# robert80203/HuPR-A-Benchmark-for-Human-Pose-Estimation-Using-Millimeter-Wave-Radar

Hardware: AMD Instinct MI355X
Metric: radar frames/sec (FFT->heatmap fwd+bwd) (higher is better)
Workload: dtype bf16

## Files before the change

### hupr-a-benchmark-for-human-pose-estimation-using-millimeter-wave-radar_amd/csrc/conv_halo256m_bf16.hip

```cpp
#include "conv_halo.h"

namespace hupr {

typedef float f32x4c __attribute__((ext_vector_type(4)));

template <int TD, int TH, int TW, int KD, int NCOT = 0, int NWN = 2, int KC = 64, bool TP = false>
__global__ __launch_bounds__(512) void hupr_k_conv_halo256m_bf16(HaloArgs p) {
    constexpr int LDK = KC, BN = 32 * NWN, TS = KC == 64 ? 3 : 9, C8 = KC / 8, L2C8 = KC == 64 ? 3 : 2;
    static_assert(KC == 64 || (KC == 32 && KD == 3 && NWN == 2 && NCOT == 0), "32-channel rows: 3 x 3 x 3 taps, 64 output channels per tile");
    static_assert(!TP || (TD == 2 && KD == 3 && NWN == 2 && KC == 64), "two-plane form: the 2 x 8 x 16 tile at D == 2 (launcher: nd == 1)");
    constexpr int NIMG = TP ? 2 * TS : TS;
    constexpr int HD = TP ? TD : TD + KD - 1, HH = TH + 2, HW = TW + 2;
    static_assert(TD * TH * TW == 64 * (8 / NWN) && TH % 8 == 0 && TW % 8 == 0 && (KD == 1 || KD == 3) && (NWN == 2 || NCOT == 0),
                  "256 (512) voxels per tile, 8 x 8 per wave");
    constexpr int NVOX = HD * HH * HW;
    constexpr int T = 9 * KD, NSTAGE = TP ? 6 : (KC == 64 ? 3 * KD : KD), NTAP = KC == 64 ? 6 : 9;
    constexpr bool FULLD = NWN == 1;
    constexpr int NVOXL = FULLD ? TD * HH * HW : NVOX, VOX0 = FULLD ? HH * HW : 0;
    constexpr int NH = (NVOXL * C8 + 511) / 512;
    constexpr int Y0 = NH < NTAP - 1 ? NH : NTAP - 1, Y1 = NH - (NTAP - 1) < 0 ? 0 : (NH - (NTAP - 1) > NTAP ? NTAP : NH - (NTAP - 1)),
                  Y2 = NH - (2 * NTAP - 1) < 0 ? 0 : (NH - (2 * NTAP - 1) > NTAP ? NTAP : NH - (2 * NTAP - 1));
    static_assert(NH <= NTAP * NSTAGE - 1 && NH <= 3 * NTAP - 1, "halo items must all be issued in front of the item's last barrier (and within three stages)");
    __shared__ __attribute__((aligned(16))) __bf16 Hs[(KC == 32 ? 2 : 1) * NVOX * LDK];
    __shared__ __attribute__((aligned(16))) __bf16 Bs[2][NIMG][BN * LDK];
    constexpr bool STATS = NCOT > 0 && KD == 3;
    constexpr bool SINGLE = STATS && TD == 2;
    f32x4c ssum[STATS ? NCOT : 1][2], ssq[STATS ? NCOT : 1][2];
    if constexpr (!SINGLE) {
#pragma unroll
        for (int ct = 0; ct < (STATS ? NCOT : 1); ++ct)
#pragma unroll
            for (int cg = 0; cg < 2; ++cg) { ssum[ct][cg] = (f32x4c){0.f, 0.f, 0.f, 0.f}; ssq[ct][cg] = (f32x4c){0.f, 0.f, 0.f, 0.f}; }
    }

    const int tid = threadIdx.x, lane = tid & 63, wave = tid >> 6;
    if (wave >= 4) __builtin_amdgcn_s_setprio(1);
    const int wm = NWN == 2 ? wave >> 1 : wave, wn = NWN == 2 ? wave & 1 : 0;
    constexpr int NBX = TW / 8, NBY = TH / 8;
    const int xw0 = 8 * (wm % NBX), yw0 = 8 * ((wm / NBX) % NBY), dzw = wm / (NBX * NBY);
    const int idx = lane & 15, kq = lane >> 4, yy = idx >> 3, wx = idx & 7;
    const int n_tiles = p.Bn * p.nd * p.nh * p.nw * p.n_co_tiles;

    const int wrow_ = NWN == 2 ? 8 * wave + (lane >> 3) : ((8 * wave + (lane >> 3)) & 31);
    const int wsrc_lane = (wrow_ * T * p.Ci + (((lane & 7) ^ (wrow_ >> 1)) & 7) * 8) * 2 +
                          (NWN == 2 ? 0 : (wave >> 2) * (3 * p.Ci * 2));
    constexpr int NDMA = NWN == 2 ? NIMG : 2, DMA_TAPS = NWN == 2 ? 1 : 2;
    const int wrow32_ = 16 * (wave & 3) + (lane >> 2);
    const int wsrc32_lane = (wrow32_ * T * p.Ci + (((lane & 3) ^ (((wrow32_ >> 3) & 1) << 1)) & 3) * 8) * 2;
    const u32x4 wrs = {(unsigned)(unsigned long)p.wp, (unsigned)((unsigned long)p.wp >> 32) & 0xffffu,
                       (unsigned)((long)p.Co * T * p.Ci * 2), 0x00020000u};
    const unsigned bs_lds = (unsigned)(unsigned long)(__attribute__((address_space(3))) void*)&Bs[0][0][0];
    const unsigned wdst_wave = __builtin_amdgcn_readfirstlane(bs_lds + wave * 1024);
#define HUPR_W_DMA(COT_, CH_, S_, PAR_)                                                                             \
    if constexpr (KC == 32) {                                                                                       \
        _Pragma("unroll") for (int j = 0; j < 5; ++j) {                                                             \
            if (j < 4 || wave < 4) {                                                                                \
                const int t9_ = 2 * j + (wave >> 2);                                  \
                const int wb32_ = (((COT_) * BN * T + (S_) * 9 + (t9_ % 3) * 3 + t9_ / 3) * p.Ci + (CH_) * KC) * 2 + wsrc32_lane; \
                unsigned keep_;                                                                                     \
                asm volatile("s_mov_b32 %0, m0\n\ts_mov_b32 m0, %1\n\ts_nop 0\n\tbuffer_load_dwordx4 %2, %3, 0 offen lds\n\t" \
                             "s_mov_b32 m0, %0"                                                                     \
                             : "=&s"(keep_)                                                                         \
                             : "s"(wdst_wave + (PAR_) * TS * (BN * LDK * 2) + j * 8192), "v"(wb32_), "s"(wrs)       \
                             : "memory");                                                                           \
            }                                                                                                       \
        }                                                                                                           \
    } else {                                                                                                        \
        const int wbase_ = (((COT_) * BN * T + ((S_) / 3) * 9 + ((S_) % 3)) * p.Ci + (CH_) * KC) * 2 + wsrc_lane;   \
        _Pragma("unroll") for (int j = 0; j < NDMA; ++j) {                                                          \
            if (NWN == 2 || j == 0 || wave < 4) {                                                                   \
                 \
                               \
                const int tap_ = (j < 3 ? 9 : 0) + 3 * (j % 3);                                                     \
                unsigned keep_;                                                                                     \
                asm volatile("s_mov_b32 %0, m0\n\ts_mov_b32 m0, %1\n\ts_nop 0\n\tbuffer_load_dwordx4 %2, %3, 0 offen lds\n\t" \
                             "s_mov_b32 m0, %0"                                                                     \
                             : "=&s"(keep_)                                                                         \
                             : "s"(NWN == 2 ? wdst_wave + ((PAR_) * NIMG + j) * (BN * LDK * 2)                      \
                                            : wdst_wave + (PAR_) * TS * (BN * LDK * 2) + j * 8192),                 \
                               "v"(TP ? wbase_ + tap_ * (p.Ci * 2)                                                  \
                                      : (NWN == 2 ? wbase_ + j * (3 * p.Ci * 2) : wbase_ + j * DMA_TAPS * (3 * p.Ci * 2))), "s"(wrs) \
                             : "memory");                                                                           \
            }                                                                                                       \
        }                                                                                                           \
    }

    u32x4 vb[NH];
    const __amdgpu_buffer_rsrc_t xrs = __builtin_amdgcn_make_buffer_rsrc(
        const_cast<void*>(p.x), 0, (int)((long)p.Bn * p.D * p.H * p.W * p.in_ld * 2), 0x00020000);
#define HUPR_HALO_ISSUE_ITEM(u, COND_, B_, D0_, H0_, W0_, C0_)                                                     \
    {                                                                                                               \
        const int it = tid + (u) * 512;                                                                             \
        const int vox = it >> L2C8, c8 = it & (C8 - 1);                                                             \
        const int hx = vox % HW;                                                                                    \
        const int t_ = vox / HW;                                                                                    \
        const int hy = t_ % HH, hz = t_ / HH;                                                                       \
        const int d = (D0_) + hz - (FULLD || TP ? 0 : KD / 2), h = (H0_) + hy - 1, w = (W0_) + hx - 1;                    \
        const bool ok = (COND_) && it < NVOXL * C8 && (unsigned)d < (unsigned)p.D && (unsigned)h < (unsigned)p.H && \
                        (unsigned)w < (unsigned)p.W;                                                                \
        const int off = (((((B_) * p.D + d) * p.H + h) * p.W + w) * p.in_ld + (C0_) + c8 * 8) * 2;                  \
        const auto ld_ = __builtin_amdgcn_raw_buffer_load_b128(xrs, ok ? off : 0x7ffffff0, 0, 0);                  \
        vb[u] = (u32x4){ld_[0], ld_[1], ld_[2], ld_[3]};                                                            \
    }
#define HUPR_HALO_COMMIT()                                                                                          \
    _Pragma("unroll") for (int u = 0; u < NH; ++u) {                                                                \
        const int it = tid + u * 512;                                                                               \
        if (it < NVOXL * C8) {                                                                                      \
            const int vox = it >> L2C8, c8 = it & (C8 - 1);                                                         \
            const int hx = vox % HW;                                                                                \
            const int key_ = KC == 64 ? (((hx >> 1) & 3) << 1) : ((((vox / HW) % HH) & 1) << 1);                    \
            *reinterpret_cast<u32x4*>(&Hs[(vox + VOX0) * LDK + ((c8 ^ key_) << 3)]) = vb[u];                        \
        }                                                                                                           \
    }

    struct Pos { int cot, twi, thi, tdi, b, ch; };
    const int n_chunks = p.Ci / KC;
    const int per_wg = (n_tiles + gridDim.x - 1) / gridDim.x;
    const int wg_rank = (int)((blockIdx.x & 7) * (gridDim.x >> 3) + (blockIdx.x >> 3));
    const int t_begin = wg_rank * per_wg, t_end = min(n_tiles, t_begin + per_wg);
    if (STATS && p.stats) {
        if (t_begin >= t_end) {
            for (int c = tid; c < 2 * p.Co; c += 512) p.stats[(long)blockIdx.x * 2 * p.Co + c] = 0.0;
        }
    }
    if (t_begin >= t_end) return;
    Pos cur;
    {
        cur.cot = t_begin % p.n_co_tiles;
        int st = t_begin / p.n_co_tiles;
        cur.twi = st % p.nw; st /= p.nw;
        cur.thi = st % p.nh; st /= p.nh;
        cur.tdi = st % p.nd;
        cur.b = st / p.nd;
        cur.ch = 0;
    }
    const int n_items = (t_end - t_begin) * n_chunks;
    const int cot0 = cur.cot;

    int woff[2][2];
#pragma unroll
    for (int cg = 0; cg < 2; ++cg)
#pragma unroll
        for (int kk = 0; kk < 2; ++kk) {
            const int n = 32 * wn + 16 * cg + idx;
            woff[cg][kk] = KC == 64 ? n * LDK + (((4 * kk + kq) ^ ((n >> 1) & 7)) << 3) : n * LDK + ((kq ^ (((n >> 3) & 1) << 1)) << 3);
            if constexpr (TP) woff[cg][kk] += dzw * (TS * BN * LDK);
        }
    const int xlane = (((TP ? 0 : dzw) * HH + yw0 + yy) * HW + xw0 + wx) * LDK;
#define HUPR_HALO_COMMIT1(u, HW_)                                                                                   \
    {                                                                                                               \
        const int it = tid + (u) * 512;                                                                             \
        if (it < NVOXL * C8) {                                                                                      \
            const int vox = it >> L2C8, c8 = it & (C8 - 1);                                                         \
            const int key_ = (((vox / HW) % HH) & 1) << 1;                                                          \
            *reinterpret_cast<u32x4*>(&Hs[(HW_) + (vox + VOX0) * LDK + ((c8 ^ key_) << 3)]) = vb[u];                \
        }                                                                                                           \
    }
#define HUPR_XF(ST_, RHO_, KK_)                                                                                     \
    (KC == 64 ? *reinterpret_cast<const bf16x8*>(&Hs[xlane + ((((ST_) / 3) * HH + (RHO_)) * HW + ((ST_) % 3)) * LDK + \
                    (((4 * (KK_) + kq) ^ ((((xw0 + wx + ((ST_) % 3)) >> 1) & 3) << 1)) << 3)])                      \
              : *reinterpret_cast<const bf16x8*>(&Hs[hrd + xlane + (((ST_) * HH + (RHO_)) * HW + (KK_)) * LDK +     \
                    ((kq ^ (((yy + (RHO_)) & 1) << 1)) << 3)]))
#define HUPR_WF(BUF_, KY_, CG_, KK_)                                                                                \
    (TP ? *reinterpret_cast<const bf16x8*>(&Bs[0][0][0] + ((BUF_) * NIMG + (KY_)) * (BN * LDK) + woff[CG_][KK_])    \
     : KC == 64 ? *reinterpret_cast<const bf16x8*>(&Bs[BUF_][KY_][woff[CG_][KK_]])                                  \
              : *reinterpret_cast<const bf16x8*>(&Bs[BUF_][3 * (KK_) + (KY_)][woff[CG_][0]]))

    f32x4c c[4][2];
    unsigned accP[4][2][2];
    __bf16* pP = nullptr;
    bool pend = false;
    constexpr bool RESPF = !STATS && TD != 2 && NWN == 2;
    const bool res_pf = RESPF && p.res != nullptr && (p.res_ld & 3) == 0 && !p.no_res_prefetch;
    constexpr bool BIASPF = KC == 32;
    const bool defer = (!p.bias || BIASPF) && (!p.res || res_pf) && (p.Co & 7) == 0 && (p.out_ld & 7) == 0;
    float biasv[BIASPF ? 2 : 1][4];
    bf16x4 resv[4][2];
    constexpr int NB = KC == 64 ? 2 : 3;
    bf16x8 xq[NB][4], x8, wq[NB][2];
#define HUPR_LOAD_TAP(ST_, TAU_, BUF_, WX_)                                                                         \
    {                                                                                                               \
        constexpr int kk_ = (TAU_) / 3, ky_ = (TAU_) % 3;                                                           \
        if ((WX_) & 1) {                                                                                            \
            wq[(TAU_) % NB][0] = HUPR_WF(BUF_, ky_, 0, kk_);                                                        \
            wq[(TAU_) % NB][1] = HUPR_WF(BUF_, ky_, 1, kk_);                                                        \
        }                                                                                                           \
        if ((WX_) & 2) {                                                                                            \
            if (ky_ == 0) { _Pragma("unroll") for (int vg = 0; vg < 4; ++vg) xq[kk_ % NB][vg] = HUPR_XF(ST_, 2 * vg, kk_); } \
            else if (ky_ == 1) { _Pragma("unroll") for (int vg = 0; vg < 4; ++vg) xq[(kk_ + 1) % NB][vg] = HUPR_XF(ST_, 2 * vg + 1, kk_); } \
            else { x8 = HUPR_XF(ST_, 8, kk_); }                                                                     \
        }                                                                                                           \
    }
#define HUPR_VMCNT_LGKM0(N_) __builtin_amdgcn_s_waitcnt(0x0070 | ((N_) & 15) | (((N_) >> 4) << 14))

    if constexpr (FULLD) {
        for (int i = tid; i < 2 * HH * HW * C8; i += 512) {
            const int pl = i / (HH * HW * C8), r = i - pl * (HH * HW * C8);
            *reinterpret_cast<u32x4*>(&Hs[pl * (HD - 1) * HH * HW * LDK + r * 8]) = (u32x4){0u, 0u, 0u, 0u};
        }
    }
    HUPR_W_DMA(cur.cot, cur.ch, 0, 0)
    HUPR_W_DMA(cur.cot, cur.ch, 1, 1)
#pragma unroll
    for (int u = 0; u < NH; ++u) HUPR_HALO_ISSUE_ITEM(u, true, cur.b, cur.tdi * TD, cur.thi * TH, cur.twi * TW, cur.ch * KC)
    [[maybe_unused]] int hrd = 0;
    if constexpr (KC == 32) {
#pragma unroll
        for (int u = 0; u < NH; ++u) HUPR_HALO_COMMIT1(u, 0)
    } else {
        HUPR_HALO_COMMIT()
    }
    __builtin_amdgcn_s_waitcnt(0x0F70);
    __syncthreads();
    HUPR_LOAD_TAP(0, 0, 0, 3)

    int g = 0;
    for (int q = 0; q < n_items; ++q) {
        const int b = cur.b, d0 = cur.tdi * TD, h0 = cur.thi * TH, w0 = cur.twi * TW, n0 = cur.cot * BN;
        const bool first_chunk = cur.ch == 0, last_chunk = cur.ch == n_chunks - 1;
        Pos nxt = cur;
        if (++nxt.ch == n_chunks) {
            nxt.ch = 0;
            if (++nxt.cot == p.n_co_tiles) {
                nxt.cot = 0;
                if (++nxt.twi == p.nw) {
                    nxt.twi = 0;
                    if (++nxt.thi == p.nh) {
                        nxt.thi = 0;
                        if (++nxt.tdi == p.nd) { nxt.tdi = 0; ++nxt.b; }
                    }
                }
            }
        }
        const bool has_next = q + 1 < n_items;
        if constexpr (KC == 32) hrd = (q & 1) * (NVOX * LDK);
        [[maybe_unused]] const int hwr = NVOX * LDK - hrd;
        if (first_chunk) {
#pragma unroll
            for (int vg = 0; vg < 4; ++vg)
#pragma unroll
                for (int cg = 0; cg < 2; ++cg) c[vg][cg] = (f32x4c){0.f, 0.f, 0.f, 0.f};
            if constexpr (BIASPF) {
                if (p.bias && defer) {
#pragma unroll
                    for (int cg = 0; cg < 2; ++cg)
#pragma unroll
                        for (int r = 0; r < 4; ++r) biasv[cg][r] = p.bias[n0 + 32 * wn + 16 * cg + 4 * kq + r];
                }
            }
        }
#pragma unroll
        for (int st_ = 0; st_ < NSTAGE; ++st_) {
            const int par = TP ? (st_ & 1) : ((g + st_) & 1);
#pragma unroll
            for (int tau = 0; tau < NTAP; ++tau) {
                const int kk = tau / 3, ky = tau % 3;
                if (tau == NTAP - 1) {
                    if (st_ == 0) { if (pend) { HUPR_VMCNT_LGKM0(Y0 + 4); } else { HUPR_VMCNT_LGKM0(Y0); } }
                    else if (st_ == 1) { HUPR_VMCNT_LGKM0(Y1); }
                    else if (st_ == 2) { HUPR_VMCNT_LGKM0(Y2); }
                    else { HUPR_VMCNT_LGKM0(0); }
                    __syncthreads();
                    if (st_ + 2 < NSTAGE) { HUPR_W_DMA(cur.cot, cur.ch, st_ + 2, par) }
                    else if (has_next) { HUPR_W_DMA(nxt.cot, nxt.ch, st_ + 2 - NSTAGE, par) }
                    if (KC == 64 && st_ == NSTAGE - 1 && has_next) { HUPR_HALO_COMMIT() }
                }
                if (tau == 0) { HUPR_LOAD_TAP(st_, 1, par, 3) }
                else if (tau == 1) { HUPR_LOAD_TAP(st_, 2, par, 3) }
                else if (tau == 2) { HUPR_LOAD_TAP(st_, 3, par, 3) }
                else if (tau == 3) { HUPR_LOAD_TAP(st_, 4, par, 3) }
                else if (tau == 4) { HUPR_LOAD_TAP(st_, 5, par, 3) }
                else if (NTAP == 9 && tau == 5) { if constexpr (NTAP == 9) { HUPR_LOAD_TAP(st_, 6, par, 3) } }
                else if (NTAP == 9 && tau == 6) { if constexpr (NTAP == 9) { HUPR_LOAD_TAP(st_, 7, par, 3) } }
                else if (NTAP == 9 && tau == 7) { if constexpr (NTAP == 9) { HUPR_LOAD_TAP(st_, 8, par, 3) } }
                else if (st_ + 1 < NSTAGE) { HUPR_LOAD_TAP((st_ + 1) % NSTAGE, 0, par ^ 1, 3) }
                else if (has_next) {
                    if constexpr (KC == 32) { const int hrd = hwr; HUPR_LOAD_TAP(0, 0, par ^ 1, 3) }
                    else { HUPR_LOAD_TAP(0, 0, par ^ 1, 1) }
                }
#pragma unroll
                for (int vg = 0; vg < 4; ++vg) {
                    const bf16x8 xf = ky == 0 ? xq[kk % NB][vg] : (ky == 1 ? xq[(kk + 1) % NB][vg] : (vg < 3 ? xq[kk % NB][vg + 1] : x8));
                    c[vg][0] = __builtin_amdgcn_mfma_f32_16x16x32_bf16(wq[tau % NB][0], xf, c[vg][0], 0, 0, 0);
                    c[vg][1] = __builtin_amdgcn_mfma_f32_16x16x32_bf16(wq[tau % NB][1], xf, c[vg][1], 0, 0, 0);
                }
                if (st_ == 0 && pend && tau < 4) {
                    const auto r0 = __builtin_amdgcn_permlane16_swap(accP[tau][0][0], accP[tau][1][0], false, false);
                    const auto r1 = __builtin_amdgcn_permlane16_swap(accP[tau][0][1], accP[tau][1][1], false, false);
                    *reinterpret_cast<u32x4*>(pP + (long)(2 * tau * p.W) * p.out_ld) = (u32x4){r0[0], r1[0], r0[1], r1[1]};
                }
                if (RESPF && st_ == NSTAGE - 1 && tau == 0) {
                    if (res_pf && last_chunk && defer) {
                        const long mr = (((long)b * p.D + d0 + dzw) * p.H + h0 + yw0 + yy) * p.W + w0 + xw0 + wx;
                        const int chr = n0 + 32 * wn + 4 * kq;
#pragma unroll
                        for (int vg = 0; vg < 4; ++vg)
#pragma unroll
                            for (int cg = 0; cg < 2; ++cg)
                                resv[vg][cg] = *reinterpret_cast<const bf16x4*>(static_cast<const __bf16*>(p.res) + (mr + 2 * vg * p.W) * p.res_ld +
                                                                                chr + 16 * cg);
                    }
                }
                if constexpr (KC == 32) {
                    if (st_ == NSTAGE - 1 && tau < NH && has_next) { HUPR_HALO_COMMIT1(tau, hwr) }
                }
                if (NTAP * st_ + tau < NH) {
                    HUPR_HALO_ISSUE_ITEM(NTAP * st_ + tau, has_next, nxt.b, nxt.tdi * TD, nxt.thi * TH, nxt.twi * TW, nxt.ch * KC)
                }
                __builtin_amdgcn_sched_group_barrier(0x100, 1, 0);
                __builtin_amdgcn_sched_group_barrier(0x008, 2, 0);
                __builtin_amdgcn_sched_group_barrier(0x100, 1, 0);
                __builtin_amdgcn_sched_group_barrier(0x008, 2, 0);
#pragma unroll
                for (int i_ = 0; i_ < 4; ++i_) {
                    __builtin_amdgcn_sched_group_barrier(0x100, 1, 0);
                    __builtin_amdgcn_sched_group_barrier(0x008, 1, 0);
                }
                __builtin_amdgcn_sched_barrier(0);
            }
            if (st_ == 0) pend = false;
        }
        g += NSTAGE;
        if (last_chunk) {
            const long m0 = (((long)b * p.D + d0 + dzw) * p.H + h0 + yw0 + yy) * p.W + w0 + xw0 + wx;
            const int ch0 = n0 + 32 * wn + 4 * kq;
            typedef __bf16 bf16x2 __attribute__((ext_vector_type(2)));
            if (defer && has_next) {
                if constexpr (BIASPF) {
                    if (p.bias) {
#pragma unroll
                        for (int vg = 0; vg < 4; ++vg)
#pragma unroll
                            for (int cg = 0; cg < 2; ++cg)
#pragma unroll
                                for (int r = 0; r < 4; ++r) c[vg][cg][r] += biasv[cg][r];
                    }
                }
                if (RESPF && res_pf) {
#pragma unroll
                    for (int vg = 0; vg < 4; ++vg)
#pragma unroll
                        for (int cg = 0; cg < 2; ++cg)
#pragma unroll
                            for (int r = 0; r < 4; ++r) c[vg][cg][r] += (float)resv[vg][cg][r];
                }
#pragma unroll
                for (int vg = 0; vg < 4; ++vg)
#pragma unroll
                    for (int cg = 0; cg < 2; ++cg) {
                        const bf16x2 lo = {(__bf16)c[vg][cg][0], (__bf16)c[vg][cg][1]}, hi = {(__bf16)c[vg][cg][2], (__bf16)c[vg][cg][3]};
                        accP[vg][cg][0] = __builtin_bit_cast(unsigned, lo);
                        accP[vg][cg][1] = __builtin_bit_cast(unsigned, hi);
                    }
                pP = static_cast<__bf16*>(p.y) + m0 * p.out_ld + n0 + 32 * wn + ((kq & 1) ? 16 + 4 * (kq - 1) : 4 * kq);
                pend = true;
            } else {
#pragma unroll
                for (int vg = 0; vg < 4; ++vg)
#pragma unroll
                    for (int cg = 0; cg < 2; ++cg) {
                        const long m = m0 + 2 * vg * p.W;
                        const int ch = ch0 + 16 * cg;
                        if (ch < p.Co) {
                            f32x4n v = {c[vg][cg][0], c[vg][cg][1], c[vg][cg][2], c[vg][cg][3]};
                            if (p.bias) v += (f32x4n){p.bias[ch], p.bias[ch + 1], p.bias[ch + 2], p.bias[ch + 3]};
                            if (p.res) {
                                const bf16x4 rv = *reinterpret_cast<const bf16x4*>(static_cast<const __bf16*>(p.res) + m * p.res_ld + ch);
                                v += (f32x4n){(float)rv[0], (float)rv[1], (float)rv[2], (float)rv[3]};
                            }
                            const bf16x4 o = {(__bf16)v[0], (__bf16)v[1], (__bf16)v[2], (__bf16)v[3]};
                            *reinterpret_cast<bf16x4*>(static_cast<__bf16*>(p.y) + m * p.out_ld + ch) = o;
                        }
                    }
            }
            if (STATS && p.stats) {
                int li = cur.cot - cot0;
                li += li < 0 ? p.n_co_tiles : 0;
                if constexpr (SINGLE) {
#pragma unroll
                    for (int cg = 0; cg < 2; ++cg) {
                        f32x4c sv = {0.f, 0.f, 0.f, 0.f}, qv = sv;
#pragma unroll
                        for (int vg = 0; vg < 4; ++vg)
#pragma unroll
                            for (int r = 0; r < 4; ++r) {
                                const float a = (float)(__bf16)c[vg][cg][r];
                                sv[r] += a;
                                qv[r] = fmaf(a, a, qv[r]);
                            }
                        ssum[0][cg] = sv;
                        ssq[0][cg] = qv;
                    }
                } else {
#pragma unroll
                    for (int ct = 0; ct < NCOT; ++ct)
                        if (NCOT == 1 || li == ct) {
#pragma unroll
                            for (int cg = 0; cg < 2; ++cg)
#pragma unroll
                                for (int vg = 0; vg < 4; ++vg)
#pragma unroll
                                    for (int r = 0; r < 4; ++r) {
                                        const float a = (float)(__bf16)c[vg][cg][r];
                                        ssum[ct][cg][r] += a;
                                        ssq[ct][cg][r] = fmaf(a, a, ssq[ct][cg][r]);
                                    }
                        }
                }
            }
        }
        if (KC == 64 && has_next) {
            __syncthreads();
            HUPR_LOAD_TAP(0, 0, g & 1, 2)
        }
        cur = nxt;
    }
    if (STATS && p.stats) {
        static_assert(NVOX * LDK * 2 >= 8 * 64 * 16 * 4, "the halo image must hold the reduction scratch");
        float (*St)[64][16] = reinterpret_cast<float (*)[64][16]>(Hs);
#pragma unroll
        for (int ct = 0; ct < NCOT; ++ct) {
            __syncthreads();
#pragma unroll
            for (int cg = 0; cg < 2; ++cg) {
                *reinterpret_cast<f32x4c*>(&St[wave][lane][4 * cg]) = ssum[ct][cg];
                *reinterpret_cast<f32x4c*>(&St[wave][lane][8 + 4 * cg]) = ssq[ct][cg];
            }
            __syncthreads();
            if (tid < 2 * BN) {
                const int k = tid >> 6, ch = tid & 63;
                const int wn_ = ch >> 5, cg = (ch >> 4) & 1, kq_ = (ch >> 2) & 3, r = ch & 3;
                double t = 0.0;
#pragma unroll
                for (int wm_ = 0; wm_ < 4; ++wm_)
#pragma unroll
                    for (int i = 0; i < 16; ++i) t += (double)St[2 * wm_ + wn_][16 * kq_ + i][8 * k + 4 * cg + r];
                p.stats[(long)blockIdx.x * 2 * p.Co + k * p.Co + 64 * ((cot0 + ct) % p.n_co_tiles) + ch] = t;
            }
        }
        if (tid < 2 * BN) {
            const int k = tid >> 6, ch = tid & 63;
            for (int ct = NCOT; ct < p.n_co_tiles; ++ct)
                p.stats[(long)blockIdx.x * 2 * p.Co + k * p.Co + 64 * ((cot0 + ct) % p.n_co_tiles) + ch] = 0.0;
        }
    }
#undef HUPR_W_DMA
#undef HUPR_HALO_ISSUE_ITEM
#undef HUPR_HALO_COMMIT
#undef HUPR_HALO_COMMIT1
#undef HUPR_XF
#undef HUPR_WF
#undef HUPR_LOAD_TAP
#undef HUPR_VMCNT_LGKM0
}

static int g_halo_two_plane = 1;
void set_halo_two_plane(int on) { g_halo_two_plane = on; }

void launch_conv_halo256(const HaloArgs& a, int route, hipStream_t s) {
    const dim3 grid(kHalo256Grid), wg(512);
    const bool tp = g_halo_two_plane && a.TD == 2 && a.D == 2 && a.nd == 1;
    switch (route) {
    case kRouteCi32: HUPR_LAUNCH((hupr_k_conv_halo256m_bf16<4, 8, 8, 3, 0, 2, 32>), grid, wg, 0, s, a); break;
    case kRouteCo32: HUPR_LAUNCH((hupr_k_conv_halo256m_bf16<8, 8, 8, 3, 0, 1>), grid, wg, 0, s, a); break;
    case kRoute1x16x16: HUPR_LAUNCH((hupr_k_conv_halo256m_bf16<1, 16, 16, 1>), grid, wg, 0, s, a); break;
    case kRouteStats4x8x8One: HUPR_LAUNCH((hupr_k_conv_halo256m_bf16<4, 8, 8, 3, 1>), grid, wg, 0, s, a); break;
    case kRouteStats4x8x8Two: HUPR_LAUNCH((hupr_k_conv_halo256m_bf16<4, 8, 8, 3, 2>), grid, wg, 0, s, a); break;
    case kRouteStats2x8x16:
        if (tp) HUPR_LAUNCH((hupr_k_conv_halo256m_bf16<2, 8, 16, 3, 1, 2, 64, true>), grid, wg, 0, s, a);
        else HUPR_LAUNCH((hupr_k_conv_halo256m_bf16<2, 8, 16, 3, 1>), grid, wg, 0, s, a);
        break;
    case kRoute4x8x8: HUPR_LAUNCH((hupr_k_conv_halo256m_bf16<4, 8, 8, 3>), grid, wg, 0, s, a); break;
    case kRoute2x8x16:
        if (tp) HUPR_LAUNCH((hupr_k_conv_halo256m_bf16<2, 8, 16, 3, 0, 2, 64, true>), grid, wg, 0, s, a);
        else HUPR_LAUNCH((hupr_k_conv_halo256m_bf16<2, 8, 16, 3>), grid, wg, 0, s, a);
        break;
    }
}

static int g_halo_tiles = 31;
void set_halo_tiles(int mask) { g_halo_tiles = mask & 31; }

static bool offsets_fit(const HaloArgs& a, int Bn) { return (long)Bn * a.D * a.H * a.W * a.in_ld * 2 < 0x7ffffff0L; }

bool conv_halo256_supported(const HaloArgs& a, int Bn, bool abf) {
    if (!abf || !(g_halo_tiles & 1)) return false;
    if (a.kd != 3 || a.D % 4 != 0 || a.H % 8 != 0 || a.W % 8 != 0 || a.Ci % 64 != 0 || a.Co % 64 != 0) return false;
    const long tiles = (long)Bn * (a.D / 4) * (a.H / 8) * (a.W / 8) * (a.Co / 64);
    if (tiles >= (1L << 31) || tiles < 256) return false;
    return offsets_fit(a, Bn);
}

bool conv_halo256_stats_ok(const HaloArgs& a, int Bn) {
    if (a.kd != 3 || a.Ci % 64 != 0 || a.Co % 64 != 0 || !offsets_fit(a, Bn)) return false;
    const int n = a.Co / 64;
    if (a.D % 4 == 0) {
        if (!conv_halo256_supported(a, Bn, true)) return false;
        if (n == 1) return true;
        const long tiles = (long)Bn * (a.D / 4) * (a.H / 8) * (a.W / 8) * n;
        const long per_wg = (tiles + kHalo256Grid - 1) / kHalo256Grid;
        return n <= 2 || per_wg == 1;
    }
    if (!(g_halo_tiles & 2) || a.D % 2 != 0 || a.H % 8 != 0 || a.W % 16 != 0) return false;
    return (long)Bn * (a.D / 2) * (a.H / 8) * (a.W / 16) * n == 256;
}

int conv_halo256_route(HaloArgs& a, int Bn, bool abf) {
    if (!abf || !offsets_fit(a, Bn)) return 0;
    if (a.Ci == 32) {
        if (!(g_halo_tiles & 16) || a.kd != 3 || a.D % 4 != 0 || a.H % 8 != 0 || a.W % 8 != 0 || a.Co % 64 != 0 || a.stats ||
            (a.in_ld & 7) || (long)a.Co * 27 * a.Ci * 2 >= 0x7ffffff0L)
            return 0;
        a.n_co_tiles = a.Co / 64;
        a.TD = 4; a.log2TW = 3;
        a.nd = a.D / 4; a.nh = a.H / 8; a.nw = a.W / 8;
        const long tiles_ = (long)Bn * a.nd * a.nh * a.nw * a.n_co_tiles;
        if (tiles_ < 256 || tiles_ >= (1L << 31)) return 0;
        return kRouteCi32;
    }
    if (a.Ci % 64 != 0) return 0;
    if (a.Co == 32) {
        if (!(g_halo_tiles & 8) || a.kd != 3 || a.D != 8 || a.H % 8 != 0 || a.W % 8 != 0 || a.stats || (a.out_ld & 7)) return 0;
        a.n_co_tiles = 1;
        a.TD = 8; a.log2TW = 3;
        a.nd = a.D / 8; a.nh = a.H / 8; a.nw = a.W / 8;
        const long tiles32 = (long)Bn * a.nd * a.nh * a.nw;
        if (tiles32 < 256 || tiles32 >= (1L << 31)) return 0;
        return kRouteCo32;
    }
    if (a.Co % 64 != 0) return 0;
    a.n_co_tiles = a.Co / 64;
    if (a.kd == 3 && a.D % 4 == 0) {
        if (!conv_halo256_supported(a, Bn, abf)) return 0;
        a.TD = 4; a.log2TW = 3;
        a.nd = a.D / 4; a.nh = a.H / 8; a.nw = a.W / 8;
    } else if (a.kd == 3) {
        if (!(g_halo_tiles & 2) || a.D % 2 != 0 || a.H % 8 != 0 || a.W % 16 != 0) return 0;
        a.TD = 2; a.log2TW = 4;
        a.nd = a.D / 2; a.nh = a.H / 8; a.nw = a.W / 16;
    } else {
        if (!(g_halo_tiles & 4) || a.kd != 1 || a.D != 1 || a.H % 16 != 0 || a.W % 16 != 0 || a.stats) return 0;
        a.TD = 1; a.log2TW = 4;
        a.nd = 1; a.nh = a.H / 16; a.nw = a.W / 16;
    }
    const long tiles = (long)Bn * a.nd * a.nh * a.nw * a.n_co_tiles;
    if (tiles < 256 || tiles >= (1L << 31)) return 0;
    if (a.TD == 1) return kRoute1x16x16;
    if (a.stats) {
        const long per_wg = (tiles + kHalo256Grid - 1) / kHalo256Grid;
        if (a.TD == 4) return (per_wg == 1 || a.n_co_tiles == 1) ? kRouteStats4x8x8One : kRouteStats4x8x8Two;
        return kRouteStats2x8x16;
    }
    return a.TD == 4 ? kRoute4x8x8 : kRoute2x8x16;
}

}
```

Measured before the change: 1803.

## Add slice-pair wave mapping to skip zero-padded depth taps in 4x8x8 halo conv

Adds a DS template variant of the 4x8x8 halo convolution in which each wave covers two depth slices by four rows instead of one slice by eight rows. The tap loop becomes a macro body instantiated in variants, so waves whose slice pair touches the depth boundary skip the MFMAs and LDS loads for padded depth taps. The launcher selects it by default when D == 4 and nd == 1, or when mask bit 64 is set. This adds code size and control-flow variants, and changes the LDS read pattern and the output and residual addressing.

```diff
diff --git a/hupr-a-benchmark-for-human-pose-estimation-using-millimeter-wave-radar_amd/csrc/conv_halo256m_bf16.hip b/hupr-a-benchmark-for-human-pose-estimation-using-millimeter-wave-radar_amd/csrc/conv_halo256m_bf16.hip
--- a/hupr-a-benchmark-for-human-pose-estimation-using-millimeter-wave-radar_amd/csrc/conv_halo256m_bf16.hip
+++ b/hupr-a-benchmark-for-human-pose-estimation-using-millimeter-wave-radar_amd/csrc/conv_halo256m_bf16.hip
@@ -4,11 +4,12 @@
 
 typedef float f32x4c __attribute__((ext_vector_type(4)));
 
-template <int TD, int TH, int TW, int KD, int NCOT = 0, int NWN = 2, int KC = 64, bool TP = false>
+template <int TD, int TH, int TW, int KD, int NCOT = 0, int NWN = 2, int KC = 64, bool TP = false, bool DS = false>
 __global__ __launch_bounds__(512) void hupr_k_conv_halo256m_bf16(HaloArgs p) {
     constexpr int LDK = KC, BN = 32 * NWN, TS = KC == 64 ? 3 : 9, C8 = KC / 8, L2C8 = KC == 64 ? 3 : 2;
     static_assert(KC == 64 || (KC == 32 && KD == 3 && NWN == 2 && NCOT == 0), "32-channel rows: 3 x 3 x 3 taps, 64 output channels per tile");
     static_assert(!TP || (TD == 2 && KD == 3 && NWN == 2 && KC == 64), "two-plane form: the 2 x 8 x 16 tile at D == 2 (launcher: nd == 1)");
+    static_assert(!DS || (TD == 4 && TH == 8 && TW == 8 && KD == 3 && NWN == 2 && KC == 64 && !TP), "slice-pair form: the 4 x 8 x 8 tile, 64-channel rows");
     constexpr int NIMG = TP ? 2 * TS : TS;
     constexpr int HD = TP ? TD : TD + KD - 1, HH = TH + 2, HW = TW + 2;
     static_assert(TD * TH * TW == 64 * (8 / NWN) && TH % 8 == 0 && TW % 8 == 0 && (KD == 1 || KD == 3) && (NWN == 2 || NCOT == 0),
@@ -37,7 +38,9 @@
     if (wave >= 4) __builtin_amdgcn_s_setprio(1);
     const int wm = NWN == 2 ? wave >> 1 : wave, wn = NWN == 2 ? wave & 1 : 0;
     constexpr int NBX = TW / 8, NBY = TH / 8;
-    const int xw0 = 8 * (wm % NBX), yw0 = 8 * ((wm / NBX) % NBY), dzw = wm / (NBX * NBY);
+    constexpr int YS = DS ? 2 : 1;
+    const int xw0 = 8 * (wm % NBX), yw0 = DS ? 4 * (wm & 1) : 8 * ((wm / NBX) % NBY), dzw = DS ? 2 * (wm >> 1) : wm / (NBX * NBY);
+#define HUPR_VGOFF(VG_) (DS ? ((VG_) >> 1) * (p.H * p.W) + ((VG_) & 1) * p.W : 2 * (VG_) * p.W)
     const int idx = lane & 15, kq = lane >> 4, yy = idx >> 3, wx = idx & 7;
     const int n_tiles = p.Bn * p.nd * p.nh * p.nw * p.n_co_tiles;
 
@@ -146,7 +149,7 @@
             woff[cg][kk] = KC == 64 ? n * LDK + (((4 * kk + kq) ^ ((n >> 1) & 7)) << 3) : n * LDK + ((kq ^ (((n >> 3) & 1) << 1)) << 3);
             if constexpr (TP) woff[cg][kk] += dzw * (TS * BN * LDK);
         }
-    const int xlane = (((TP ? 0 : dzw) * HH + yw0 + yy) * HW + xw0 + wx) * LDK;
+    const int xlane = (((TP ? 0 : dzw) * HH + yw0 + YS * yy) * HW + xw0 + wx) * LDK;
 #define HUPR_HALO_COMMIT1(u, HW_)                                                                                   \
     {                                                                                                               \
         const int it = tid + (u) * 512;                                                                             \
@@ -166,6 +169,7 @@
      : KC == 64 ? *reinterpret_cast<const bf16x8*>(&Bs[BUF_][KY_][woff[CG_][KK_]])                                  \
               : *reinterpret_cast<const bf16x8*>(&Bs[BUF_][3 * (KK_) + (KY_)][woff[CG_][0]]))
 
+    [[maybe_unused]] const int dzs = DS ? __builtin_amdgcn_readfirstlane(dzw) : 0;
     f32x4c c[4][2];
     unsigned accP[4][2][2];
     __bf16* pP = nullptr;
@@ -178,20 +182,89 @@
     bf16x4 resv[4][2];
     constexpr int NB = KC == 64 ? 2 : 3;
     bf16x8 xq[NB][4], x8, wq[NB][2];
-#define HUPR_LOAD_TAP(ST_, TAU_, BUF_, WX_)                                                                         \
+#define HUPR_LOAD_TAP(ST_, TAU_, BUF_, WX_, LM_)                                                                    \
     {                                                                                                               \
         constexpr int kk_ = (TAU_) / 3, ky_ = (TAU_) % 3;                                                           \
         if ((WX_) & 1) {                                                                                            \
             wq[(TAU_) % NB][0] = HUPR_WF(BUF_, ky_, 0, kk_);                                                        \
             wq[(TAU_) % NB][1] = HUPR_WF(BUF_, ky_, 1, kk_);                                                        \
         }                                                                                                           \
-        if ((WX_) & 2) {                                                                                            \
+        if (DS && ((WX_) & 2)) {                                                                                    \
+            _Pragma("unroll") for (int s_ = 0; s_ < 2; ++s_) {                                                      \
+                if ((LM_) == s_ + 1) continue;                                                                      \
+                if (ky_ == 0) { _Pragma("unroll") for (int vl = 0; vl < 2; ++vl) xq[s_][vl] = HUPR_XF(ST_, s_ * HH + vl, kk_); } \
+                else { xq[s_][ky_ + 1] = HUPR_XF(ST_, s_ * HH + ky_ + 1, kk_); }                                    \
+            }                                                                                                       \
+        } else if ((WX_) & 2) {                                                                                     \
             if (ky_ == 0) { _Pragma("unroll") for (int vg = 0; vg < 4; ++vg) xq[kk_ % NB][vg] = HUPR_XF(ST_, 2 * vg, kk_); } \
             else if (ky_ == 1) { _Pragma("unroll") for (int vg = 0; vg < 4; ++vg) xq[(kk_ + 1) % NB][vg] = HUPR_XF(ST_, 2 * vg + 1, kk_); } \
             else { x8 = HUPR_XF(ST_, 8, kk_); }                                                                     \
         }                                                                                                           \
     }
 #define HUPR_VMCNT_LGKM0(N_) __builtin_amdgcn_s_waitcnt(0x0070 | ((N_) & 15) | (((N_) >> 4) << 14))
+
+#define HUPR_TAP_BODY(MM_, LM_)                                                                                     \
+    {                                                                                                               \
+        \
+        if (tau == 0) { HUPR_LOAD_TAP(st_, 1, par, 3, LM_) }                                                        \
+        else if (tau == 1) { HUPR_LOAD_TAP(st_, 2, par, 3, LM_) }                                                   \
+        else if (tau == 2) { HUPR_LOAD_TAP(st_, 3, par, 3, LM_) }                                                   \
+        else if (tau == 3) { HUPR_LOAD_TAP(st_, 4, par, 3, LM_) }                                                   \
+        else if (tau == 4) { HUPR_LOAD_TAP(st_, 5, par, 3, LM_) }                                                   \
+        else if (NTAP == 9 && tau == 5) { if constexpr (NTAP == 9) { HUPR_LOAD_TAP(st_, 6, par, 3, LM_) } }         \
+        else if (NTAP == 9 && tau == 6) { if constexpr (NTAP == 9) { HUPR_LOAD_TAP(st_, 7, par, 3, LM_) } }         \
+        else if (NTAP == 9 && tau == 7) { if constexpr (NTAP == 9) { HUPR_LOAD_TAP(st_, 8, par, 3, LM_) } }         \
+        else if (st_ + 1 < NSTAGE) { HUPR_LOAD_TAP((st_ + 1) % NSTAGE, 0, par ^ 1, 3, LM_) }                        \
+        else if (has_next) {                                                                                        \
+            if constexpr (KC == 32) { const int hrd = hwr; HUPR_LOAD_TAP(0, 0, par ^ 1, 3, LM_) }      \
+            else { HUPR_LOAD_TAP(0, 0, par ^ 1, 1, LM_) }                                                           \
+        }                                                                                                           \
+        \
+        _Pragma("unroll") for (int vg = 0; vg < 4; ++vg) {                                                          \
+            if (!DS || (MM_) != (vg >> 1) + 1) {                                                                    \
+                const bf16x8 xf = DS ? xq[vg >> 1][(vg & 1) + ky] : ky == 0 ? xq[kk % NB][vg] : (ky == 1 ? xq[(kk + 1) % NB][vg] : (vg < 3 ? xq[kk % NB][vg + 1] : x8));\
+                c[vg][0] = __builtin_amdgcn_mfma_f32_16x16x32_bf16(wq[tau % NB][0], xf, c[vg][0], 0, 0, 0);         \
+                c[vg][1] = __builtin_amdgcn_mfma_f32_16x16x32_bf16(wq[tau % NB][1], xf, c[vg][1], 0, 0, 0);         \
+            }                                                                                                       \
+        }                                                                                                           \
+        if (st_ == 0 && pend && tau < 4) {                                                                          \
+            \
+            \
+            \
+            const auto r0 = __builtin_amdgcn_permlane16_swap(accP[tau][0][0], accP[tau][1][0], false, false);       \
+            const auto r1 = __builtin_amdgcn_permlane16_swap(accP[tau][0][1], accP[tau][1][1], false, false);       \
+            *reinterpret_cast<u32x4*>(pP + (long)HUPR_VGOFF(tau) * p.out_ld) = (u32x4){r0[0], r1[0], r0[1], r1[1]}; \
+        }                                                                                                           \
+        if (RESPF && st_ == NSTAGE - 1 && tau == 0) {                                                               \
+            if (res_pf && last_chunk && defer) {                                                                    \
+                const long mr = (((long)b * p.D + d0 + dzw) * p.H + h0 + yw0 + YS * yy) * p.W + w0 + xw0 + wx;           \
+                const int chr = n0 + 32 * wn + 4 * kq;                                                              \
+                _Pragma("unroll") for (int vg = 0; vg < 4; ++vg)                                                    \
+                    _Pragma("unroll") for (int cg = 0; cg < 2; ++cg)                                                \
+                        resv[vg][cg] = *reinterpret_cast<const bf16x4*>(static_cast<const __bf16*>(p.res) + (mr + HUPR_VGOFF(vg)) * p.res_ld +\
+                                                                        chr + 16 * cg);                             \
+            }                                                                                                       \
+        }                                                                                                           \
+        if constexpr (KC == 32) {                         \
+            if (st_ == NSTAGE - 1 && tau < NH && has_next) { HUPR_HALO_COMMIT1(tau, hwr) }                          \
+        }                                                                                                           \
+        \
+        if (NTAP * st_ + tau < NH) {                                                                                \
+            HUPR_HALO_ISSUE_ITEM(NTAP * st_ + tau, has_next, nxt.b, nxt.tdi * TD, nxt.thi * TH, nxt.twi * TW, nxt.ch * KC)\
+        }                                                                                                           \
+        \
+        if ((MM_) == 0) {                                                                                           \
+            __builtin_amdgcn_sched_group_barrier(0x100, 1, 0);                                                      \
+            __builtin_amdgcn_sched_group_barrier(0x008, 2, 0);                                                      \
+            __builtin_amdgcn_sched_group_barrier(0x100, 1, 0);                                                      \
+            __builtin_amdgcn_sched_group_barrier(0x008, 2, 0);                                                      \
+        }                                                                                                           \
+        _Pragma("unroll") for (int i_ = 0; i_ < 4; ++i_) {                                                          \
+            __builtin_amdgcn_sched_group_barrier(0x100, 1, 0);                                                      \
+            __builtin_amdgcn_sched_group_barrier(0x008, 1, 0);                                                      \
+        }                                                                                                           \
+        __builtin_amdgcn_sched_barrier(0);                                                                          \
+    }
 
     if constexpr (FULLD) {
         for (int i = tid; i < 2 * HH * HW * C8; i += 512) {
@@ -212,7 +285,7 @@
     }
     __builtin_amdgcn_s_waitcnt(0x0F70);
     __syncthreads();
-    HUPR_LOAD_TAP(0, 0, 0, 3)
+    HUPR_LOAD_TAP(0, 0, 0, 3, 0)
 
     int g = 0;
     for (int q = 0; q < n_items; ++q) {
@@ -233,6 +306,7 @@
             }
         }
         const bool has_next = q + 1 < n_items;
+        [[maybe_unused]] const bool skA = DS && d0 + dzs == 0, skB = DS && d0 + dzs + 2 == p.D;
         if constexpr (KC == 32) hrd = (q & 1) * (NVOX * LDK);
         [[maybe_unused]] const int hwr = NVOX * LDK - hrd;
         if (first_chunk) {
@@ -265,64 +339,25 @@
                     else if (has_next) { HUPR_W_DMA(nxt.cot, nxt.ch, st_ + 2 - NSTAGE, par) }
                     if (KC == 64 && st_ == NSTAGE - 1 && has_next) { HUPR_HALO_COMMIT() }
                 }
-                if (tau == 0) { HUPR_LOAD_TAP(st_, 1, par, 3) }
-                else if (tau == 1) { HUPR_LOAD_TAP(st_, 2, par, 3) }
-                else if (tau == 2) { HUPR_LOAD_TAP(st_, 3, par, 3) }
-                else if (tau == 3) { HUPR_LOAD_TAP(st_, 4, par, 3) }
-                else if (tau == 4) { HUPR_LOAD_TAP(st_, 5, par, 3) }
-                else if (NTAP == 9 && tau == 5) { if constexpr (NTAP == 9) { HUPR_LOAD_TAP(st_, 6, par, 3) } }
-                else if (NTAP == 9 && tau == 6) { if constexpr (NTAP == 9) { HUPR_LOAD_TAP(st_, 7, par, 3) } }
-                else if (NTAP == 9 && tau == 7) { if constexpr (NTAP == 9) { HUPR_LOAD_TAP(st_, 8, par, 3) } }
-                else if (st_ + 1 < NSTAGE) { HUPR_LOAD_TAP((st_ + 1) % NSTAGE, 0, par ^ 1, 3) }
-                else if (has_next) {
-                    if constexpr (KC == 32) { const int hrd = hwr; HUPR_LOAD_TAP(0, 0, par ^ 1, 3) }
-                    else { HUPR_LOAD_TAP(0, 0, par ^ 1, 1) }
-                }
-#pragma unroll
-                for (int vg = 0; vg < 4; ++vg) {
-                    const bf16x8 xf = ky == 0 ? xq[kk % NB][vg] : (ky == 1 ? xq[(kk + 1) % NB][vg] : (vg < 3 ? xq[kk % NB][vg + 1] : x8));
-                    c[vg][0] = __builtin_amdgcn_mfma_f32_16x16x32_bf16(wq[tau % NB][0], xf, c[vg][0], 0, 0, 0);
-                    c[vg][1] = __builtin_amdgcn_mfma_f32_16x16x32_bf16(wq[tau % NB][1], xf, c[vg][1], 0, 0, 0);
-                }
-                if (st_ == 0 && pend && tau < 4) {
-                    const auto r0 = __builtin_amdgcn_permlane16_swap(accP[tau][0][0], accP[tau][1][0], false, false);
-                    const auto r1 = __builtin_amdgcn_permlane16_swap(accP[tau][0][1], accP[tau][1][1], false, false);
-                    *reinterpret_cast<u32x4*>(pP + (long)(2 * tau * p.W) * p.out_ld) = (u32x4){r0[0], r1[0], r0[1], r1[1]};
-                }
-                if (RESPF && st_ == NSTAGE - 1 && tau == 0) {
-                    if (res_pf && last_chunk && defer) {
-                        const long mr = (((long)b * p.D + d0 + dzw) * p.H + h0 + yw0 + yy) * p.W + w0 + xw0 + wx;
-                        const int chr = n0 + 32 * wn + 4 * kq;
-#pragma unroll
-                        for (int vg = 0; vg < 4; ++vg)
-#pragma unroll
-                            for (int cg = 0; cg < 2; ++cg)
-                                resv[vg][cg] = *reinterpret_cast<const bf16x4*>(static_cast<const __bf16*>(p.res) + (mr + 2 * vg * p.W) * p.res_ld +
-                                                                                chr + 16 * cg);
+                if constexpr (!DS) {
+                    HUPR_TAP_BODY(0, 0)
+                } else {
+                    const int mm_st = st_ < 3 ? 1 : (st_ >= 6 ? 2 : 0);
+                    const bool half = mm_st == 1 ? skA : (mm_st == 2 ? skB : false);
+#pragma unroll
+                    for (int var_ = 0; var_ < 2; ++var_) {
+                        if (var_ == 0 ? half : !half) continue;
+                        const int mm = var_ ? mm_st : 0;
+                        const int lm = (tau < NTAP - 1 || (st_ + 1 < NSTAGE && (st_ + 1 < 3 ? 1 : (st_ + 1 >= 6 ? 2 : 0)) == mm)) ? mm : 0;
+                        HUPR_TAP_BODY(mm, lm)
                     }
                 }
-                if constexpr (KC == 32) {
-                    if (st_ == NSTAGE - 1 && tau < NH && has_next) { HUPR_HALO_COMMIT1(tau, hwr) }
-                }
-                if (NTAP * st_ + tau < NH) {
-                    HUPR_HALO_ISSUE_ITEM(NTAP * st_ + tau, has_next, nxt.b, nxt.tdi * TD, nxt.thi * TH, nxt.twi * TW, nxt.ch * KC)
-                }
-                __builtin_amdgcn_sched_group_barrier(0x100, 1, 0);
-                __builtin_amdgcn_sched_group_barrier(0x008, 2, 0);
-                __builtin_amdgcn_sched_group_barrier(0x100, 1, 0);
-                __builtin_amdgcn_sched_group_barrier(0x008, 2, 0);
-#pragma unroll
-                for (int i_ = 0; i_ < 4; ++i_) {
-                    __builtin_amdgcn_sched_group_barrier(0x100, 1, 0);
-                    __builtin_amdgcn_sched_group_barrier(0x008, 1, 0);
-                }
-                __builtin_amdgcn_sched_barrier(0);
             }
             if (st_ == 0) pend = false;
         }
         g += NSTAGE;
         if (last_chunk) {
-            const long m0 = (((long)b * p.D + d0 + dzw) * p.H + h0 + yw0 + yy) * p.W + w0 + xw0 + wx;
+            const long m0 = (((long)b * p.D + d0 + dzw) * p.H + h0 + yw0 + YS * yy) * p.W + w0 + xw0 + wx;
             const int ch0 = n0 + 32 * wn + 4 * kq;
             typedef __bf16 bf16x2 __attribute__((ext_vector_type(2)));
             if (defer && has_next) {
@@ -359,7 +394,7 @@
                 for (int vg = 0; vg < 4; ++vg)
 #pragma unroll
                     for (int cg = 0; cg < 2; ++cg) {
-                        const long m = m0 + 2 * vg * p.W;
+                        const long m = m0 + HUPR_VGOFF(vg);
                         const int ch = ch0 + 16 * cg;
                         if (ch < p.Co) {
                             f32x4n v = {c[vg][cg][0], c[vg][cg][1], c[vg][cg][2], c[vg][cg][3]};
@@ -411,7 +446,7 @@
         }
         if (KC == 64 && has_next) {
             __syncthreads();
-            HUPR_LOAD_TAP(0, 0, g & 1, 2)
+            HUPR_LOAD_TAP(0, 0, g & 1, 2, 0)
         }
         cur = nxt;
     }
@@ -445,32 +480,46 @@
         }
     }
 #undef HUPR_W_DMA
+#undef HUPR_VGOFF
 #undef HUPR_HALO_ISSUE_ITEM
 #undef HUPR_HALO_COMMIT
 #undef HUPR_HALO_COMMIT1
 #undef HUPR_XF
 #undef HUPR_WF
 #undef HUPR_LOAD_TAP
+#undef HUPR_TAP_BODY
 #undef HUPR_VMCNT_LGKM0
 }
 
 static int g_halo_two_plane = 1;
 void set_halo_two_plane(int on) { g_halo_two_plane = on; }
+static int g_halo_tiles = 31;
+void set_halo_tiles(int mask) { g_halo_tiles = mask & 127; }
 
 void launch_conv_halo256(const HaloArgs& a, int route, hipStream_t s) {
     const dim3 grid(kHalo256Grid), wg(512);
     const bool tp = g_halo_two_plane && a.TD == 2 && a.D == 2 && a.nd == 1;
+    const bool ds = a.TD == 4 && ((g_halo_tiles & 64) || (!(g_halo_tiles & 32) && a.D == 4 && a.nd == 1));
     switch (route) {
     case kRouteCi32: HUPR_LAUNCH((hupr_k_conv_halo256m_bf16<4, 8, 8, 3, 0, 2, 32>), grid, wg, 0, s, a); break;
     case kRouteCo32: HUPR_LAUNCH((hupr_k_conv_halo256m_bf16<8, 8, 8, 3, 0, 1>), grid, wg, 0, s, a); break;
     case kRoute1x16x16: HUPR_LAUNCH((hupr_k_conv_halo256m_bf16<1, 16, 16, 1>), grid, wg, 0, s, a); break;
-    case kRouteStats4x8x8One: HUPR_LAUNCH((hupr_k_conv_halo256m_bf16<4, 8, 8, 3, 1>), grid, wg, 0, s, a); break;
-    case kRouteStats4x8x8Two: HUPR_LAUNCH((hupr_k_conv_halo256m_bf16<4, 8, 8, 3, 2>), grid, wg, 0, s, a); break;
+    case kRouteStats4x8x8One:
+        if (ds) HUPR_LAUNCH((hupr_k_conv_halo256m_bf16<4, 8, 8, 3, 1, 2, 64, false, true>), grid, wg, 0, s, a);
+        else HUPR_LAUNCH((hupr_k_conv_halo256m_bf16<4, 8, 8, 3, 1>), grid, wg, 0, s, a);
+        break;
+    case kRouteStats4x8x8Two:
+        if (ds) HUPR_LAUNCH((hupr_k_conv_halo256m_bf16<4, 8, 8, 3, 2, 2, 64, false, true>), grid, wg, 0, s, a);
+        else HUPR_LAUNCH((hupr_k_conv_halo256m_bf16<4, 8, 8, 3, 2>), grid, wg, 0, s, a);
+        break;
     case kRouteStats2x8x16:
         if (tp) HUPR_LAUNCH((hupr_k_conv_halo256m_bf16<2, 8, 16, 3, 1, 2, 64, true>), grid, wg, 0, s, a);
         else HUPR_LAUNCH((hupr_k_conv_halo256m_bf16<2, 8, 16, 3, 1>), grid, wg, 0, s, a);
         break;
-    case kRoute4x8x8: HUPR_LAUNCH((hupr_k_conv_halo256m_bf16<4, 8, 8, 3>), grid, wg, 0, s, a); break;
+    case kRoute4x8x8:
+        if (ds) HUPR_LAUNCH((hupr_k_conv_halo256m_bf16<4, 8, 8, 3, 0, 2, 64, false, true>), grid, wg, 0, s, a);
+        else HUPR_LAUNCH((hupr_k_conv_halo256m_bf16<4, 8, 8, 3>), grid, wg, 0, s, a);
+        break;
     case kRoute2x8x16:
         if (tp) HUPR_LAUNCH((hupr_k_conv_halo256m_bf16<2, 8, 16, 3, 0, 2, 64, true>), grid, wg, 0, s, a);
         else HUPR_LAUNCH((hupr_k_conv_halo256m_bf16<2, 8, 16, 3>), grid, wg, 0, s, a);
@@ -478,8 +527,6 @@
     }
 }
 
-static int g_halo_tiles = 31;
-void set_halo_tiles(int mask) { g_halo_tiles = mask & 31; }
 
 static bool offsets_fit(const HaloArgs& a, int Bn) { return (long)Bn * a.D * a.H * a.W * a.in_ld * 2 < 0x7ffffff0L; }
 
```

Result: no change. 1811, median of 6 (+0.4%).
